# patrickzbhe/ray-tracing-series-rust

Hardware: AMD Instinct MI355X
Metric: Msamples/s (pixels x spp) on Book-1 final scene (higher is better)
Workload: dtype f64

## Files before the change

### ray-tracing-series-rust_amd/csrc/hip/pass_items.inc

```

struct ShardMap {
  int32_t width, block_rows, shard_index, shard_count;
};
struct ActiveMap : ShardMap {
  const uint32_t* active;
};
__device__ __forceinline__ uint32_t map_pixel(const ShardMap&, uint32_t k) { return k; }
__device__ __forceinline__ uint32_t map_pixel(const ActiveMap& m, uint32_t k) { return m.active[k]; }
__device__ __forceinline__ void shard_pixel(const ShardMap& m, uint32_t lp, uint32_t* i, uint32_t* j) {
  uint32_t lr = lp / (uint32_t)m.width;
  *i = lp - lr * (uint32_t)m.width;
  uint32_t k = lr / (uint32_t)m.block_rows;
  uint32_t within = lr - k * (uint32_t)m.block_rows;
  *j = (k * (uint32_t)m.shard_count + (uint32_t)m.shard_index) * (uint32_t)m.block_rows + within;
}

template <class SM>
__device__ __forceinline__ uint32_t item_pixel(const SM& sm, uint32_t npix, uint32_t g, uint32_t* i, uint32_t* j) {
  const uint32_t s_local = g / npix;
  shard_pixel(sm, map_pixel(sm, g - s_local * npix), i, j);
  return s_local;
}

template <class SM>
__device__ __forceinline__ void start_path(const rt::RenderParams& rp, const SM& sm, uint32_t npix, uint32_t s_begin,
                                           uint32_t g, rt::PathState* ps) {
  uint32_t i, j;
  const uint32_t s_local = item_pixel(sm, npix, g, &i, &j);
  rt::path_begin(rp, i, j, s_begin + s_local, ps);
}

__device__ __forceinline__ void store_sample(double* samples, uint32_t g, const rt::Color& c) {
  double* o = samples + 3 * (size_t)g;
  o[0] = c.x; o[1] = c.y; o[2] = c.z;
}

#define TRACE_CHUNK 512u

__device__ __forceinline__ uint32_t lane_rank(unsigned long long mask) {
  return __builtin_amdgcn_mbcnt_hi((uint32_t)(mask >> 32), __builtin_amdgcn_mbcnt_lo((uint32_t)mask, 0u));
}

__device__ __forceinline__ uint32_t queue_claim(unsigned int* work_counter, uint32_t chunk) {
  uint32_t base = 0;
  if ((threadIdx.x & 63u) == 0u) base = atomicAdd(work_counter, chunk);
  return __builtin_amdgcn_readfirstlane(base);
}

#define RING_F64 9u
__host__ __device__ constexpr uint32_t ring_bytes(uint32_t cap) { return cap * (RING_F64 * 8u + 4u); }
```

### ray-tracing-series-rust_amd/csrc/hip/render.hip

```cpp
#include <hip/hip_runtime.h>
#include <cstdio>
#include <cstdlib>
#include <algorithm>
#include <chrono>
#include <cfloat>
#include <cmath>
#include <cstring>
#include <new>
#include <type_traits>
#include <utility>
#include <string>
#include <vector>
#include "../../../include/rtx_abi.h"
#include "../core/cull32.hpp"
#include "../core/integrator.hpp"
#include "../host/flat_scene.hpp"
#include "../host/light_table.hpp"
#include "device_buffer.hpp"
#include "f32_bridge.hpp"
#ifndef RTX_F32_TU
#include "abi_internal.hpp"
#else
namespace rtx { void set_error(const std::string& msg); }
#endif

namespace rtx {

#include "pass_items.inc"

struct FlatNode4;
typedef const FlatNode4 FlatNode4Dev;
struct WorldDesc;

struct LdsSceneDims {
  uint32_t n_nodes, n_refs, n_spheres, n_moving;
  uint32_t node_dwords;
  uint32_t n_uni;
};

struct VoteTop {
  int32_t n;
  int32_t all_rects;
  int32_t k[8];
  uint32_t ref[8];
  rt::FlatRect rect[8];
};

enum class ForcedKernel { none, simple, vote, world, wavefront };

struct TraceSwitches {
  ForcedKernel kernel = ForcedKernel::none;
  bool diag = false;
  int ring = -1, wide = -1, scene_lds = -1;
  bool vote_top = true, tri_direct = true, mat_lds = true, perlin_lds = true;
  bool mv_common = true, motion = true, motion_axis = true;
  bool single_leaf = true, pass_pipeline = true, validate = false;
  uint32_t chunk = TRACE_CHUNK;
  uint32_t world_threshold = 8;
  uint32_t walk_threshold = 0, regen_min = 0, leaf_weight = 0;
  uint32_t wf_paths = 1u << 22, wf_refill = 16, wf_check = 8;
  int wf_occ = 4;
  bool wf_verbose = false;
};

struct Workspace {
  DeviceBuffer<double> samples;
  DeviceBuffer<double> accum;
  DeviceBuffer<rt::TraceCounters> counters;
  DeviceBuffer<unsigned int> work_counter;
  DeviceBuffer<unsigned long long> diag;
  hipEvent_t ev[2] = {nullptr, nullptr};
  hipStream_t aux_stream = nullptr;
  hipEvent_t ev_pass[3] = {nullptr, nullptr, nullptr};
  DeviceBuffer<unsigned char> wave_mem;
  uint32_t* wave_host_ctrl = nullptr;
};

struct VotePlan {
  bool ok = false;
  int32_t bvh_pos = 0;
  int32_t tri_base = -1;
  VoteTop top;
  int blocks_per_cu[2] = {1, 1};
  bool ring[2] = {false, false};
  uint32_t tables = 0;
  size_t tables_bytes = 0;
};

struct WidePlan {
  FlatNode4Dev* nodes4 = nullptr;
  int levels = 0;
  int vote_blocks_per_cu = 1;
};

struct WorldPlan {
  const WorldDesc* desc = nullptr;
  uint32_t mat_lds = 0, tex_lds = 0;
  uint32_t perlin_lds = 0;
  int blocks_per_cu[5][2] = {{1, 1}, {1, 1}, {1, 1}, {1, 1}, {1, 1}};
};

struct LdsFit {
  bool ok = false;
  uint32_t ring_cap = 0;
  uint32_t levels = 0;
  LdsSceneDims dims = {0, 0, 0, 0, 0, 0};
};

struct LdsPlan {
  LdsFit plain;
  LdsFit motion;
  int motion_axis = -1;
  double motion_t0 = 0.0, motion_t1 = 0.0;
  bool mv_common = false;
  double mv_t0 = 0.0, mv_t1 = 1.0;
};

struct WalkTuning {
  uint32_t walk_threshold = 18;
  uint32_t regen_min = 1;
  uint32_t leaf_weight = 3;
  bool single_leaf = false;
};

struct DeviceScene {
  int device = -1;
  std::vector<DeviceBuffer<void>> allocations;
  rt::SceneView view;
  size_t scene_bytes = 0;
  int n_cu = 256;
  double gravity_time_limit = 1e300;
  TraceSwitches sw;
  Workspace ws;
  VotePlan vote;
  WidePlan wide;
  WorldPlan world;
  LdsPlan lds;
  WalkTuning walk;
  rt::LightView lights = {nullptr, nullptr, 0, 0};
};

#define HIP_TRY(expr)                                                                      \
  do {                                                                                     \
    hipError_t _e = (expr);                                                                \
    if (_e != hipSuccess) {                                                                \
      set_error(std::string(#expr) + ": " + hipGetErrorString(_e));                        \
      return RTX_EHIP;                                                                     \
    }                                                                                      \
  } while (0)

template <class T>
static rtx_status upload_array(DeviceScene* ds, const std::vector<T>& v, const T** out) {
  *out = nullptr;
  if (v.empty()) return RTX_OK;
  DeviceBuffer<void> b;
  size_t bytes = v.size() * sizeof(T);
  HIP_TRY(b.alloc(bytes));
  HIP_TRY(hipMemcpy(b, v.data(), bytes, hipMemcpyHostToDevice));
  ds->scene_bytes += bytes;
  *out = (const T*)(void*)b;
  ds->allocations.push_back(std::move(b));
  return RTX_OK;
}

static void free_device_scene(DeviceScene* ds) {
  if (!ds) return;
  Workspace& ws = ds->ws;
  if (ws.wave_host_ctrl) (void)hipHostFree(ws.wave_host_ctrl);
  for (int i = 0; i < 2; ++i)
    if (ws.ev[i]) (void)hipEventDestroy(ws.ev[i]);
  for (int i = 0; i < 3; ++i)
    if (ws.ev_pass[i]) (void)hipEventDestroy(ws.ev_pass[i]);
  if (ws.aux_stream) (void)hipStreamDestroy(ws.aux_stream);
  delete ds;
}

template <class T>
__device__ __forceinline__ T dev_load_uniform(const T* p) { return *(const __attribute__((address_space(4))) T*)(p); }

__device__ __forceinline__ unsigned long long wave_ballot(bool p) { return __builtin_amdgcn_ballot_w64(p); }

#define TRACE_BLOCK 256
struct LdsStack {
  int32_t* base;
  int n;
  static constexpr bool kBottom = false;
  __device__ __forceinline__ void reset() { n = 0; }
  __device__ __forceinline__ void push(int32_t v) { base[n * TRACE_BLOCK] = v; ++n; }
  __device__ __forceinline__ int32_t pop() { --n; return base[n * TRACE_BLOCK]; }
  __device__ __forceinline__ bool empty() const { return n == 0; }
};
// ... 275 lines not shown
  if (a.preset == 0) { LAUNCH_VOTE(P_SPHERES); }
  else { LAUNCH_VOTE(P_MESH); }
#undef LAUNCH_VOTE
#undef LAUNCH_VOTE2
#undef LAUNCH_VOTE3
  return RTX_OK;
}

static void validate_wide_tree(const FlatScene& fs, const std::vector<FlatNode4>& wide, int levels) {
  for (const rt::FlatEntry& e : fs.entries) {
    if (e.kind != rt::ENTRY_BVH) continue;
    std::vector<std::pair<int32_t, int>> todo;
    todo.push_back({e.a, 0});
    size_t visited = 0, bad = 0; int deepest = 0;
    while (!todo.empty()) {
      auto [code, below] = todo.back(); todo.pop_back();
      if (code < 0) { if (rt::leaf_first(code) + rt::leaf_count(code) > (uint32_t)e.c) ++bad; continue; }
      if ((size_t)code >= wide.size()) { ++bad; continue; }
      ++visited;
      int nk = 0;
      for (int k = 0; k < 4; ++k) if (wide[code].child[k] != 0x7fffffff) ++nk;
      deepest = std::max(deepest, below + nk);
      for (int k = 0; k < 4; ++k) if (wide[code].child[k] != 0x7fffffff) todo.push_back({wide[code].child[k], below + nk - 1});
    }
    fprintf(stderr, "[rtx] RTX_VALIDATE: BVH root %d refs %d: %zu wide nodes walked, %zu bad codes, deepest stack %d of %d levels, sizeof(real) %zu\n",
            e.a, e.c, visited, bad, deepest, levels, sizeof(rt::real));
  }
}

static rtx_status plan_wide(DeviceScene* ds, const FlatScene& fs) {
  WidePlan& p = ds->wide;
  const bool spheres_preset = (fs.features & ~P_SPHERES) == 0;
  const bool mesh_preset = !spheres_preset && (fs.features & ~P_MESH) == 0;
  const int preset = spheres_preset ? 0 : (mesh_preset ? 1 : 2);
  const bool for_vote = ds->vote.ok && mesh_preset;
  const bool for_world = !(ds->vote.ok && preset < 2) && preset >= 1;
  bool want_wide = (for_vote && fs.nodes.size() >= 4096) || (for_world && fs.nodes.size() >= 256);
  if (ds->sw.wide >= 0) want_wide = (for_vote || for_world) && ds->sw.wide != 0 && !fs.nodes.empty();
  if (fs.features & rt::F_INSTANCE) want_wide = false;
  if (!want_wide) return RTX_OK;
  std::vector<FlatNode4> wide(fs.nodes.size());
  memset(wide.data(), 0, wide.size() * sizeof(FlatNode4));
  int peak = 0;
  for (const rt::FlatEntry& e : fs.entries)
    if (e.kind == rt::ENTRY_BVH) peak = std::max(peak, build_wide_nodes(fs.nodes, e.a, &wide));
  p.levels = peak + 1;
  const size_t lds = stack_bytes((uint32_t)p.levels);
  bool ok = lds <= 64 * 1024;
  if (ok && for_vote) {
    const int nb = occupancy(k_trace_vote<P_MESH, false, false, true>, lds);
    ok = nb > 0;
    if (ok) p.vote_blocks_per_cu = nb;
  }
  if (ok) {
    rtx_status st = upload_array(ds, wide, &p.nodes4);
    if (st != RTX_OK) return st;
  }
  if (ds->sw.wide >= 0) fprintf(stderr, "[rtx] RTX_WIDE: 4-wide tree %s (%d stack levels)\n", p.nodes4 ? "on" : "off", p.levels);
  if (ds->sw.validate) validate_wide_tree(fs, wide, p.levels);
  return RTX_OK;
}

static rtx_status plan_world(DeviceScene* ds, const FlatScene& fs) {
  WorldPlan& p = ds->world;
  const TraceSwitches& sw = ds->sw;
  rtx_status st = upload_array(ds, build_world_desc(fs), &p.desc);
  if (st != RTX_OK) return st;
  for (int wd = 0; wd < 2; ++wd) {
    const uint32_t levels = (uint32_t)(wd ? ds->wide.levels : fs.max_stack + 1);
    size_t wl = stack_bytes(levels) + (size_t)WORLD_SLOT_F64 * TRACE_BLOCK * sizeof(rt::real);
    if (wl > 64 * 1024) continue;
    if ((wd != 0) == (ds->wide.nodes4 != nullptr)) {
      const size_t n_p = fs.perlins.size();
      if (n_p >= 1 && n_p <= 2 && sw.perlin_lds && wl + n_p * sizeof(rt::FlatPerlin) <= 52 * 1024) {
        p.perlin_lds = (uint32_t)n_p;
        wl += n_p * sizeof(rt::FlatPerlin);
      }
      const size_t mt = fs.materials.size() * sizeof(rt::FlatMaterial) + fs.textures.size() * sizeof(rt::FlatTexture);
      if (!fs.materials.empty() && !fs.textures.empty() && fs.materials.size() <= 64 && fs.textures.size() <= 64 && sw.mat_lds &&
          wl + mt <= 52 * 1024) {
        p.mat_lds = (uint32_t)fs.materials.size();
        p.tex_lds = (uint32_t)fs.textures.size();
        wl += mt;
      }
    }
    int n = 0;
#define WORLD_OCC(I, FEAT) if ((n = occupancy(wd ? k_trace_world<FEAT, true, WORLD_WPS> : k_trace_world<FEAT, false, WORLD_WPS>, wl)) > 0) p.blocks_per_cu[I][wd] = n
    WORLD_OCC(0, P_BOOK2); WORLD_OCC(1, P_ANY); WORLD_OCC(2, P_ALL); WORLD_OCC(3, P_NO_SPHERE_MEDIA);
#undef WORLD_OCC
    if (wd == 0 && (n = occupancy(k_trace_world<P_INST, false, WORLD_WPS>, wl)) > 0) p.blocks_per_cu[4][0] = n;
  }
  return RTX_OK;
}

static rtx_status launch_world(DeviceScene* ds, const PassArgs& a) {
  const WorldPlan& p = ds->world;
  HIP_TRY(hipMemsetAsync(a.work_counter, 0, sizeof(unsigned int), a.stream));
  const bool wide = ds->wide.nodes4 != nullptr;
  const bool book2 = (a.feat & ~P_BOOK2) == 0;
  const bool has_gravity = (a.feat & rt::F_GRAVITY_SPHERE) != 0;
  const bool no_sphere_media = (a.feat & rt::F_MEDIUM_SPHERE) == 0;
  const uint32_t levels = wide ? (uint32_t)ds->wide.levels : a.stack_levels;
  const size_t lds = stack_bytes(levels) + (size_t)WORLD_SLOT_F64 * TRACE_BLOCK * sizeof(rt::real) +
                     (size_t)p.perlin_lds * sizeof(rt::FlatPerlin) + (size_t)p.mat_lds * sizeof(rt::FlatMaterial) +
                     (size_t)p.tex_lds * sizeof(rt::FlatTexture);
  const bool inst = (a.feat & rt::F_INSTANCE) != 0;
  const int family = inst ? 4 : (has_gravity ? 2 : (book2 ? 0 : (no_sphere_media ? 3 : 1)));
  const uint32_t grid = grid_size(a.total, TRACE_BLOCK, (uint64_t)ds->n_cu * (uint64_t)p.blocks_per_cu[family][wide ? 1 : 0]);
  const rt::SceneView& v = ds->view;
#define LAUNCH_WORLD3(FEAT, WIDEF, DIAGF, MAP)                                                                               \
  hipLaunchKernelGGL(HIP_KERNEL_NAME(k_trace_world<FEAT, WIDEF, WORLD_WPS, DIAGF, decltype(MAP)>), dim3(grid), dim3(TRACE_BLOCK), lds, \
                     a.stream, v, a.rp, MAP, a.s_begin, a.total, a.npix, a.samples, a.work_counter, v.entries, v.top_level, v.spheres, \
                     v.moving_spheres, v.rects, v.triangles, v.materials, v.textures, v.refs, ds->wide.nodes4, p.desc,     \
                     ds->walk.leaf_weight, ds->sw.world_threshold, levels, p.perlin_lds, p.mat_lds, p.tex_lds,             \
                     DIAGF ? ds->ws.diag : nullptr)
#define LAUNCH_WORLD2(FEAT, WIDEF) with_map(a, [&](auto map) { LAUNCH_WORLD3(FEAT, WIDEF, false, map); })
#define LAUNCH_WORLD(FEAT) do { if (wide) { LAUNCH_WORLD2(FEAT, true); } else { LAUNCH_WORLD2(FEAT, false); } } while (0)
  if (ds->sw.kernel == ForcedKernel::world && ds->sw.diag && book2 && wide && !a.active) {
    unsigned long long h[24];
    static const char* const names[8] = {"node_step", "leaf_step", "sweep", "shade(lean)", "regen", "direct_entry(all)", "direct_entry(run)", "shade(rare)"};
    return run_diag(ds, a.stream, [&] { LAUNCH_WORLD3(P_BOOK2, true, true, a.sm); }, "world_diag", 18, names, 8, h);
  }
  if (inst) {
    if (wide) { set_error("render: a world with an instance tree has no 4-wide tree"); return RTX_EUNSUPPORTED; }
    LAUNCH_WORLD2(P_INST, false);
  }
  else if (has_gravity) { LAUNCH_WORLD(P_ALL); }
  else if (book2) { LAUNCH_WORLD(P_BOOK2); }
  else if (no_sphere_media) { LAUNCH_WORLD(P_NO_SPHERE_MEDIA); }
  else { LAUNCH_WORLD(P_ANY); }
#undef LAUNCH_WORLD
#undef LAUNCH_WORLD2
#undef LAUNCH_WORLD3
  return RTX_OK;
}

static void fit_lds(LdsFit* f, bool want_ring, uint32_t lds_max) {
  for (uint32_t cap : {64u, 48u, 0u})
    if ((want_ring || cap == 0u) && ldsk_layout(f->levels, cap, f->dims).total <= lds_max) {
      f->ok = true;
      f->ring_cap = cap;
      return;
    }
}

static rtx_status plan_lds(DeviceScene* ds, const FlatScene& fs, const LeafScan& leaves) {
  const bool single_bvh = fs.top_level.size() == 1 && fs.entries[fs.top_level[0]].kind == rt::ENTRY_BVH;
  if (!single_bvh || (fs.features & ~P_SPHERES) != 0 || fs.nodes32.size() > LDSK_MAX_NODES) return RTX_OK;
  LdsPlan& p = ds->lds;
  const TraceSwitches& sw = ds->sw;
  const uint32_t max_end = leaves.max_end, levels = (uint32_t)fs.max_stack + 1u;
  int lds_max = 0;
  (void)hipDeviceGetAttribute(&lds_max, hipDeviceAttributeMaxSharedMemoryPerBlock, ds->device);
  if (lds_max > 160 * 1024) lds_max = 160 * 1024;
  p.plain.levels = levels;
  p.plain.dims = {(uint32_t)fs.nodes32.size(), max_end, max_end, 0u, LDSK_NODE_DWORDS, 0u};
  if (!fs.moving_spheres.empty()) {
    bool same = sw.mv_common;
    for (const rt::FlatMovingSphere& ms : fs.moving_spheres)
      same = same && ms.time0 == fs.moving_spheres[0].time0 && ms.time1 == fs.moving_spheres[0].time1;
    if (same) { p.mv_common = true; p.mv_t0 = (double)fs.moving_spheres[0].time0; p.mv_t1 = (double)fs.moving_spheres[0].time1; }
  }
  if (fs.features & rt::F_MOVING_SPHERE) {
    p.plain.dims.n_uni = (uint32_t)fs.spheres.size();
    p.plain.dims.n_moving = max_end;
    p.plain.dims.n_spheres = 0u;
  }
  p.motion.levels = levels;
  p.motion.dims = p.plain.dims;
  p.motion.dims.node_dwords = LDSK_MOTION_NODE_DWORDS;
  {
    bool moves[3] = {false, false, false};
    for (const rt::FlatMotion32& m : fs.motion32)
      for (int ch = 0; ch < 2; ++ch)
        for (int a = 0; a < 3; ++a) moves[a] = moves[a] || m.dlo[ch][a] != 0.0f || m.dhi[ch][a] != 0.0f;
    if (!fs.motion32.empty() && moves[1] && !moves[0] && !moves[2] && sw.motion_axis) {
      p.motion_axis = 1;
      p.motion.dims.node_dwords = LDSK_MOTION1_NODE_DWORDS;
    }
  }
  if (leaves.max_count <= 4 && max_end <= LDSK_MAX_SLOTS && sw.scene_lds != 0 && lds_max > 0) {
    const bool want_ring = sw.ring != 0;
    fit_lds(&p.plain, want_ring, (uint32_t)lds_max);
    const rt::FlatEntry& be = fs.entries[fs.top_level[0]];
    if (p.plain.ok && !fs.motion32.empty() && (fs.features & rt::F_MOVING_SPHERE) && (double)be.f[0] < (double)be.f[1] && sw.motion) {
      p.motion_t0 = (double)be.f[0]; p.motion_t1 = (double)be.f[1];
      fit_lds(&p.motion, want_ring, (uint32_t)lds_max);
    }
  }
  if (p.plain.ok) {
    hipError_t ae = hipSuccess;
#define LDS_ATTR1(K) if (ae == hipSuccess) ae = hipFuncSetAttribute((const void*)K, hipFuncAttributeMaxDynamicSharedMemorySize, lds_max)
#define LDS_ATTR(FEAT, RINGF, MOTIONF) LDS_ATTR1((k_trace_lds<FEAT, RINGF, MOTIONF>)); LDS_ATTR1((k_trace_lds<FEAT, RINGF, MOTIONF, ActiveMap>))
    LDS_ATTR(P_SPHERES, true, 0u); LDS_ATTR(P_SPHERES, false, 0u); LDS_ATTR(P_STATIC_SPHERES, true, 0u); LDS_ATTR(P_STATIC_SPHERES, false, 0u);
    LDS_ATTR(P_SPHERES, true, 1u); LDS_ATTR(P_SPHERES, false, 1u); LDS_ATTR(P_SPHERES, true, 3u); LDS_ATTR(P_SPHERES, false, 3u);
#undef LDS_ATTR
#undef LDS_ATTR1
    if (ae != hipSuccess) { (void)hipGetLastError(); p.plain.ok = false; }
  }
  if (sw.scene_lds >= 0) {
    auto bytes = [](const LdsFit& f) { return f.ok ? ldsk_layout(f.levels, f.ring_cap, f.dims).total : 0u; };
    fprintf(stderr, "[rtx] RTX_SCENE_LDS: k_trace_lds %s (ring of %u, %u B of LDS); time-aware boxes %s (ring of %u, %u B)\n",
            p.plain.ok ? "on" : "off", p.plain.ring_cap, ldsk_layout(levels, p.plain.ring_cap, p.plain.dims).total,
            p.motion.ok ? "on" : "off", p.motion.ring_cap, bytes(p.motion));
  }
  return RTX_OK;
}

static rtx_status launch_lds(DeviceScene* ds, const PassArgs& a, const RtxCamera* cam) {
  const LdsPlan& p = ds->lds;
  HIP_TRY(hipMemsetAsync(a.work_counter, 0, sizeof(unsigned int), a.stream));
  const bool motion = p.motion.ok && (double)cam->time1 >= p.motion_t0 && (double)cam->time2 <= p.motion_t1;
  const LdsFit& f = motion ? p.motion : p.plain;
  const bool ring = f.ring_cap != 0u;
  const rt::real m_t0 = (rt::real)p.motion_t0, m_inv = (rt::real)(1.0 / (p.motion_t1 - p.motion_t0));
  const LdsKernelLayout L = ldsk_layout(f.levels, f.ring_cap, f.dims);
  const uint32_t grid = grid_size(a.total, LDSK_BLOCK, (uint64_t)ds->n_cu);
  const WalkTuning& wk = ds->walk;
#define LAUNCH_LDS2(FEAT, RINGF, MOTIONF)                                                                               \
  with_map(a, [&](auto map) {                                                                                           \
    hipLaunchKernelGGL(HIP_KERNEL_NAME(k_trace_lds<FEAT, RINGF, MOTIONF, decltype(map)>), dim3(grid), dim3(LDSK_BLOCK), L.total, \
                       a.stream, ds->view, a.rp, map, a.s_begin, a.total, a.npix, a.samples, a.work_counter, wk.leaf_weight, \
                       wk.walk_threshold | (wk.single_leaf ? 0x100u : 0u), ds->sw.chunk, f.ring_cap, f.levels, f.dims,  \
                       m_t0, m_inv, p.mv_common ? 1u : 0u, (rt::real)p.mv_t0, (rt::real)p.mv_t1);                        \
  })
#define LAUNCH_LDS(FEAT, MOTIONF) do { if (ring) { LAUNCH_LDS2(FEAT, true, MOTIONF); } else { LAUNCH_LDS2(FEAT, false, MOTIONF); } } while (0)
  if ((a.feat & ~P_STATIC_SPHERES) == 0) { LAUNCH_LDS(P_STATIC_SPHERES, 0u); }
  else if (motion && p.motion_axis == 1) { LAUNCH_LDS(P_SPHERES, 3u); }
  else if (motion) { LAUNCH_LDS(P_SPHERES, 1u); }
  else { LAUNCH_LDS(P_SPHERES, 0u); }
#undef LAUNCH_LDS
#undef LAUNCH_LDS2
  return RTX_OK;
}

template <bool COUNT>
static void launch_simple(const DeviceScene* ds, const PassArgs& a) {
  const uint32_t grid = grid_size(a.total, TRACE_BLOCK, (uint64_t)ds->n_cu * 8);
#define LAUNCH_SIMPLE2(FEAT, MAP)                                                                                       \
  hipLaunchKernelGGL(HIP_KERNEL_NAME(k_trace_simple<FEAT, COUNT, decltype(MAP)>), dim3(grid), dim3(TRACE_BLOCK), a.stack_lds, \
                     a.stream, ds->view, a.rp, MAP, a.s_begin, a.total, a.npix, a.samples, ds->ws.counters)
#define LAUNCH_SIMPLE(FEAT) with_map(a, [&](auto map) { LAUNCH_SIMPLE2(FEAT, map); })
  const bool inst = (a.feat & rt::F_INSTANCE) != 0;
  if constexpr (COUNT) {
    if (inst) { LAUNCH_SIMPLE2(P_INST, a.sm); } else { LAUNCH_SIMPLE2(P_ALL, a.sm); }
  } else {
    if (a.preset == 0) { LAUNCH_SIMPLE(P_SPHERES); }
    else if (a.preset == 1) { LAUNCH_SIMPLE(P_MESH); }
    else if (inst) { LAUNCH_SIMPLE(P_INST); }
    else { LAUNCH_SIMPLE(P_ALL); }
  }
#undef LAUNCH_SIMPLE
#undef LAUNCH_SIMPLE2
}

#ifndef RTX_F32_TU
static rtx_status launch_nee(const DeviceScene* ds, const PassArgs& a) {
  HIP_TRY(hipMemsetAsync(a.work_counter, 0, sizeof(unsigned int), a.stream));
  const int preset = (a.feat & rt::F_INSTANCE) ? 3 : ((a.feat & ~P_MESH_ROOM) == 0 ? 0 : ((a.feat & rt::F_GRAVITY_SPHERE) ? 2 : 1));
#define LAUNCH_NEE(FEAT, MAP)                                                                                                   \
  do {                                                                                                                          \
    const int nb = occupancy(k_trace_nee<FEAT, decltype(MAP)>, a.stack_lds);                                                    \
    const uint32_t grid = grid_size(a.total, TRACE_CHUNK, (uint64_t)ds->n_cu * (uint64_t)(nb > 0 ? nb : 1) * (TRACE_BLOCK / 64)); \
    hipLaunchKernelGGL(HIP_KERNEL_NAME(k_trace_nee<FEAT, decltype(MAP)>), dim3((grid + TRACE_BLOCK / 64 - 1) / (TRACE_BLOCK / 64)),     \
                       dim3(TRACE_BLOCK), a.stack_lds, a.stream, ds->view, ds->lights, a.rp, MAP, a.s_begin, a.total, a.npix,     \
                       a.samples, a.work_counter);                                                                              \
  } while (0)
  with_map(a, [&](auto map) {
    if (preset == 0) LAUNCH_NEE(P_MESH_ROOM, map);
    else if (preset == 1) LAUNCH_NEE(P_ANY, map);
    else if (preset == 3) LAUNCH_NEE(P_INST, map);
    else LAUNCH_NEE(P_ALL, map);
  });
#undef LAUNCH_NEE
  return RTX_OK;
}
#endif

static rtx_status wave_pass(DeviceScene* ds, const PassArgs& a) {
  Workspace& ws = ds->ws;
  const hipStream_t stream = a.stream;
  uint32_t P = ds->sw.wf_paths;
  if ((uint64_t)P > (uint64_t)a.total) P = a.total;
  P = (P + WF_SEG - 1u) & ~(WF_SEG - 1u);
  const uint32_t n_seg = P / WF_SEG;
  const size_t R = sizeof(rt::real);
  const size_t bytes = 64 + (size_t)P * (16 + 7 * R + 3 * R + 3 * R + R + 4 + 4 + 4 + 4) + (size_t)n_seg * 8;
  HIP_TRY(ws.wave_mem.grow(bytes, stream));
  if (!ws.wave_host_ctrl) HIP_TRY(hipHostMalloc((void**)&ws.wave_host_ctrl, 4 * sizeof(uint32_t), hipHostMallocDefault));
  WavePool pool;
  {
    unsigned char* m = ws.wave_mem;
    pool.ctrl = (uint32_t*)m; m += 64;
    pool.rng = (unsigned long long*)m; m += (size_t)P * 16;
    pool.ray = (rt::real*)m; m += (size_t)P * 7 * R;
    pool.product = (rt::real*)m; m += (size_t)P * 3 * R;
    pool.output = (rt::real*)m; m += (size_t)P * 3 * R;
    pool.hit_t = (rt::real*)m; m += (size_t)P * R;
    pool.depth = (int32_t*)m; m += (size_t)P * 4;
    pool.g = (uint32_t*)m; m += (size_t)P * 4;
    pool.hit_ref = (uint32_t*)m; m += (size_t)P * 4;
    pool.free_list = (uint32_t*)m; m += (size_t)P * 4;
    pool.n_free = (uint32_t*)m; m += (size_t)n_seg * 4;
    pool.cursor = (uint32_t*)m; m += (size_t)n_seg * 4;
    pool.P = P;
  }
  const int preset = a.preset;
  const bool wide = preset == 1 && ds->wide.nodes4 != nullptr;
  const uint32_t levels = wide ? (uint32_t)ds->wide.levels : a.stack_levels;
  const size_t lds = stack_bytes(levels);
  if (lds > 64 * 1024) { set_error("render: BVH too deep for the LDS traversal stack"); return RTX_EUNSUPPORTED; }
  const bool room = (a.feat & ~P_MESH_ROOM) == 0;
  const int occ = ds->sw.wf_occ;
  const uint32_t leaf_weight = ds->walk.leaf_weight, refill = ds->sw.wf_refill, bvh_pos = (uint32_t)ds->vote.bvh_pos;
#define WF_CASES(X)                                                                                                          \
  if (preset == 0) { X(P_SPHERES, false, 4); }                                                                               \
  else if (!wide) { X(P_MESH, false, 4); }                                                                                   \
  else if (room && occ == 5) { X(P_MESH_ROOM, true, 5); }                                                                    \
  else if (room && occ == 6) { X(P_MESH_ROOM, true, 6); }                                                                    \
  else if (room) { X(P_MESH_ROOM, true, 4); }                                                                                \
  else { X(P_MESH, true, 4); }
  int nb = 0;
  hipError_t oe = hipSuccess;
#define WF_OCC(FEAT, WIDEF, MB) oe = hipOccupancyMaxActiveBlocksPerMultiprocessor(&nb, k_wf_trace<FEAT, WIDEF, MB>, TRACE_BLOCK, lds)
  WF_CASES(WF_OCC)
#undef WF_OCC
  if (oe != hipSuccess || nb <= 0) { (void)hipGetLastError(); nb = 1; }
  const uint32_t tgrid = grid_size(P, TRACE_BLOCK, (uint64_t)ds->n_cu * (uint64_t)nb);
  hipLaunchKernelGGL(k_wf_init, dim3((P + 255u) / 256u), dim3(256), 0, stream, pool);
  uint32_t check_every = ds->sw.wf_check;
  int it = 0;
  for (;; ++it) {
    with_map(a, [&](auto map) {
      hipLaunchKernelGGL(HIP_KERNEL_NAME(k_wf_generate<decltype(map)>), dim3(n_seg), dim3(WF_SEG), 0, stream, pool, a.rp, map,
                         a.s_begin, a.total, a.npix);
    });
    if ((uint32_t)(it + 1) % check_every == 0u) {
      HIP_TRY(hipMemsetAsync(pool.ctrl, 0, 16, stream));
      hipLaunchKernelGGL(k_wf_count, dim3(256), dim3(256), 0, stream, pool);
      HIP_TRY(hipGetLastError());
      HIP_TRY(hipMemcpyAsync(ws.wave_host_ctrl, pool.ctrl, 4 * sizeof(uint32_t), hipMemcpyDeviceToHost, stream));
      HIP_TRY(hipStreamSynchronize(stream));
      if (ws.wave_host_ctrl[0] == 0u) break;
      if (ws.wave_host_ctrl[0] < P / 2u) check_every = 2;
      if (it > 100000000) { set_error("render: wavefront integrator did not converge"); return RTX_EHIP; }
    }
#define WF_LAUNCH(FEAT, WIDEF, MB)                                                                                           \
  do {                                                                                                                       \
    hipLaunchKernelGGL(HIP_KERNEL_NAME(k_wf_trace<FEAT, WIDEF, MB>), dim3(tgrid), dim3(TRACE_BLOCK), lds, stream, ds->view, pool, \
                       leaf_weight, refill, bvh_pos, ds->wide.nodes4, ds->vote.tri_base);                                    \
    hipLaunchKernelGGL(HIP_KERNEL_NAME(k_wf_shade<FEAT>), dim3(n_seg), dim3(WF_SEG), 0, stream, ds->view, pool, a.rp, a.samples, bvh_pos); \
// ... 790 lines not shown
```

### ray-tracing-series-rust_amd/csrc/hip/trace_lds.inc

```

#define LDSK_BLOCK 1024
#define LDSK_DONE (-1)
#define LDSK_NO_REF 0xFFFFFFFFu
#define LDSK_MAX_SLOTS 8190u
#define LDSK_MAX_NODES 8191u
#define LDSK_NODE_DWORDS 21u
#ifndef LDSK_NODE_BURST
#define LDSK_NODE_BURST 1
#endif
#define LDSK_MOTION_NODE_DWORDS 39u
#define LDSK_MOTION1_NODE_DWORDS 27u

struct LdsKernelLayout {
  uint32_t off_ring, off_nodes, off_refs, off_spheres, off_moving, total;
};
__host__ __device__ inline LdsKernelLayout ldsk_layout(uint32_t levels, uint32_t ring_cap, const LdsSceneDims& d) {
  LdsKernelLayout L;
  uint32_t o = levels * LDSK_BLOCK * 2u;
  o = (o + 15u) & ~15u;
  L.off_ring = o; o += (LDSK_BLOCK / 64u) * ring_bytes(ring_cap);
  L.off_nodes = o; o += (d.n_nodes * d.node_dwords * 4u + 15u) & ~15u;
  L.off_refs = o;
  L.off_spheres = o; o += (d.n_spheres * (uint32_t)sizeof(rt::FlatSphere) + 15u) & ~15u;
  L.off_moving = o; o += (d.n_moving * (uint32_t)sizeof(rt::FlatMovingSphere) + 15u) & ~15u;
  L.total = o;
  return L;
}

struct LdsStack16 {
  unsigned short* base;
  int n;
  __device__ __forceinline__ void init() { base[0] = 0xFFFFu; n = 1; }
  __device__ __forceinline__ void reset() { n = 1; }
  __device__ __forceinline__ void push(int32_t v) { base[n * LDSK_BLOCK] = (unsigned short)v; ++n; }
  __device__ __forceinline__ int32_t pop() { --n; return (int32_t)(short)base[n * LDSK_BLOCK]; }
  __device__ __forceinline__ int32_t top() const { return (int32_t)(short)base[(n - 1) * LDSK_BLOCK]; }
};
__host__ __device__ __forceinline__ int32_t ldsk_item(int32_t child) {
  if (child >= 0) return child;
  return (int32_t)(short)(unsigned short)(0x8000u | (rt::leaf_first(child) << 2) | (rt::leaf_count(child) - 1u));
}

template <uint32_t F, bool RING, uint32_t MOTION, class SM = ShardMap>
__global__ __launch_bounds__(LDSK_BLOCK) void k_trace_lds(rt::SceneView sv, rt::RenderParams rp, SM sm,
                                                          uint32_t s_begin, uint32_t total, uint32_t npix,
                                                          double* __restrict__ samples, unsigned int* work_counter,
                                                          uint32_t leaf_weight, uint32_t walk_threshold, uint32_t chunk, uint32_t ring_cap,
                                                          uint32_t stack_levels, LdsSceneDims dims, rt::real motion_t0, rt::real motion_inv_dt,
                                                          uint32_t mv_common, rt::real mv_t0, rt::real mv_t1) {
  static_assert(!MOTION || (F & rt::F_MOVING_SPHERE), "time-aware boxes only make sense with moving spheres");
  const bool single_leaf = (walk_threshold & 0x100u) != 0u;
  walk_threshold &= 0xFFu;
  constexpr bool UNI = (F & rt::F_MOVING_SPHERE) != 0;
  constexpr uint32_t FL = UNI ? (F & ~rt::F_SPHERE) : F;
  static_assert(MOTION <= 4u, "0: no slopes, 1: all axes, 2 + a: axis a only");
  constexpr uint32_t ND = MOTION == 1u ? LDSK_MOTION_NODE_DWORDS : (MOTION >= 2u ? LDSK_MOTION1_NODE_DWORDS : LDSK_NODE_DWORDS);
  constexpr uint32_t CBD = MOTION == 1u ? 19u : (MOTION >= 2u ? 13u : 10u);
  constexpr uint32_t MA = MOTION >= 2u ? MOTION - 2u : 0u;
  constexpr uint32_t CB = CBD * 4u;
  constexpr uint32_t ITEM_OFF = CB - 4u;
  static_assert((F & ~(rt::F_SPHERE | rt::F_MOVING_SPHERE | rt::F_BVH | rt::F_LAMBERTIAN | rt::F_METAL |
                       rt::F_DIELECTRIC | rt::F_CHECKER)) == 0, "k_trace_lds caches spheres and moving spheres only");
  extern __shared__ __attribute__((aligned(16))) unsigned char ldsk[];
  const LdsKernelLayout L = ldsk_layout(stack_levels, RING ? ring_cap : 0u, dims);
  const uint32_t lane = threadIdx.x & 63u;
  const rt::FlatEntry& bvh = sv.entries[sv.top_level[0]];
  const int32_t root = bvh.a | (sv.nodes32[bvh.a].axis << 13);
  const uint32_t first_ref = (uint32_t)bvh.b;

  uint32_t* const lds_nodes = (uint32_t*)(ldsk + L.off_nodes);
  rt::FlatSphere* const lds_spheres = (rt::FlatSphere*)(ldsk + L.off_spheres);
  rt::FlatMovingSphere* const lds_moving = (rt::FlatMovingSphere*)(ldsk + L.off_moving);
  {
    static_assert(sizeof(rt::FlatNode32) == 64 && offsetof(rt::FlatNode32, child) == 48 && offsetof(rt::FlatNode32, axis) == 56,
                  "the padded LDS copy assumes FlatNode32's layout");
    const uint32_t* src = (const uint32_t*)sv.nodes32;
    const uint32_t* msrc = (const uint32_t*)sv.motion32;
    for (uint32_t k = threadIdx.x; k < dims.n_nodes * 2u * CBD; k += LDSK_BLOCK) {
      const uint32_t node = k / (2u * CBD), field = k - node * (2u * CBD);
      const uint32_t c = field / CBD, r = field - c * CBD;
      uint32_t v;
      if (r < 9u) {
        const uint32_t a = r / 3u, t = r - a * 3u;
        v = MOTION ? msrc[node * 24u + (t == 1u ? 6u : 0u) + c * 3u + a]
                   : src[node * 16u + (t == 1u ? 6u : 0u) + c * 3u + a];
      } else if (MOTION == 1u && r < 18u) {
        const uint32_t a = (r - 9u) / 3u, t = (r - 9u) - a * 3u;
        v = msrc[node * 24u + (t == 1u ? 18u : 12u) + c * 3u + a];
      } else if (MOTION >= 2u && r < 12u) {
        const uint32_t t = r - 9u;
        v = msrc[node * 24u + (t == 1u ? 18u : 12u) + c * 3u + MA];
      } else {
        const int32_t child = (int32_t)src[node * 16u + 12u + c];
        int32_t item = ldsk_item(child);
        if (child >= 0) item |= sv.nodes32[child].axis << 13;
        v = (uint32_t)item;
      }
      lds_nodes[node * ND + field] = v;
    }
    if (UNI) {
      for (uint32_t k = threadIdx.x; k < dims.n_refs; k += LDSK_BLOCK) {
        const rt::PrimRef ref = sv.refs[first_ref + k];
        rt::FlatMovingSphere m;
        if (rt::primref_type(ref) == rt::PRIM_SPHERE) {
          const rt::FlatSphere sp = sv.spheres[rt::primref_index(ref)];
          m.c0[0] = sp.cx; m.c0[1] = sp.cy; m.c0[2] = sp.cz; m.c1[0] = sp.cx; m.c1[1] = sp.cy; m.c1[2] = sp.cz;
          m.time0 = rt::real(0.0); m.time1 = rt::real(1.0); m.radius = sp.radius; m.mat = sp.mat; m.pad = 0;
        } else {
          m = sv.moving_spheres[rt::primref_index(ref)];
        }
        lds_moving[k] = m;
      }
    } else {
      constexpr uint32_t SD = (uint32_t)(sizeof(rt::FlatSphere) / 4);
      uint32_t* ds = (uint32_t*)lds_spheres;
      const uint32_t* ss = (const uint32_t*)sv.spheres;
      for (uint32_t k = threadIdx.x; k < dims.n_refs * SD; k += LDSK_BLOCK) {
        const uint32_t slot = k / SD, field = k - slot * SD;
        ds[k] = ss[rt::primref_index(sv.refs[first_ref + slot]) * SD + field];
      }
    }
  }
  __syncthreads();
  rt::SceneView lsv = sv;
  lsv.spheres = lds_spheres;
  lsv.moving_spheres = lds_moving;

  LdsStack16 stack;
  stack.base = (unsigned short*)ldsk + threadIdx.x;
  stack.init();
  double* const ring_f = (double*)(ldsk + L.off_ring + (threadIdx.x >> 6) * ring_bytes(ring_cap));
  uint32_t* const ring_g = (uint32_t*)(ring_f + RING_F64 * ring_cap);
  uint32_t ring_n = 0;
  uint32_t chunk_pos = 0, chunk_end = 0;
  bool queue_empty = false;
  bool active = false;
  uint32_t g = 0;
  rt::PathState ps;
  bool midwalk = false;
  rt::Ray32 q = {0.f, 0.f, 0.f, 0.f, 0.f, 0.f, 0.f, 0.f};
  uint32_t dir_neg = 0;
  uint32_t off_x = 0, off_y = 12, off_z = 24;
  uint32_t flip_b = 0;
  float t_max32 = 0.f;
  float s32 = 0.f;
  rt::real mv_ratio = rt::real(0.0);
  int32_t cur = LDSK_DONE;
  rt::Closest best;
  best.t = 0.0; best.ref = LDSK_NO_REF; best.order = 0; best.hit = false;

  for (;;) {
    const unsigned long long need_mask = wave_ballot(!active);
    if (need_mask != 0ull) {
      const uint32_t n_need = (uint32_t)__popcll(need_mask);
      const uint32_t rank = lane_rank(need_mask);
      if (RING) {
#define RING_CAP ring_cap
#define RING_DIAG(mask)
#include "trace_ring.inc"
#undef RING_DIAG
#undef RING_CAP
      } else {
        if (chunk_pos >= chunk_end && !queue_empty) {
          uint32_t base = 0;
          if (lane == 0) base = atomicAdd(work_counter, chunk);
          base = __builtin_amdgcn_readfirstlane(base);
          if (base >= total) {
            queue_empty = true;
          } else {
            chunk_pos = base;
            chunk_end = (total - base < chunk) ? total : base + chunk;
          }
        }
        if (chunk_pos < chunk_end) {
          const uint32_t avail = chunk_end - chunk_pos;
          if (!active && rank < avail) {
            g = chunk_pos + rank;
            start_path(rp, sm, npix, s_begin, g, &ps);
            active = true;
          }
          chunk_pos += (n_need < avail) ? n_need : avail;
        }
      }
    }
    if (wave_ballot(active) == 0ull) break;
    if (active && !midwalk) {
      if (rt::path_bounce_begin(&ps)) {
        store_sample(samples, g, ps.output);
        active = false;
      } else {
        q = rt::make_ray32(ps.ray, rt::ray_t_min(ps.ray));
        dir_neg = rt::ray_dir_neg(ps.ray);
        off_x = (dir_neg & 1u) << 2; off_y = 12u + ((dir_neg & 2u) << 1); off_z = 24u + (dir_neg & 4u);
        flip_b = ((dir_neg & 1u) * CB) | (((dir_neg >> 1) & 1u) * (CB << 8)) | (((dir_neg >> 2) & 1u) * (CB << 16));
        t_max32 = __builtin_huge_valf();
        if (UNI && mv_common != 0u) mv_ratio = (ps.ray.time - mv_t0) / (mv_t1 - mv_t0);
        if (MOTION) s32 = __builtin_fminf(__builtin_fmaxf((float)((ps.ray.time - motion_t0) * motion_inv_dt), 0.f), 1.f);
        best.t = RT_INFINITY; best.ref = LDSK_NO_REF; best.order = 0;
        stack.reset();
        cur = root;
        midwalk = true;
      }
    }
    const uint32_t threshold = (queue_empty && ring_n == 0u) ? 1u : walk_threshold;
    auto node_step = [&]() {
      const unsigned char* nd = (const unsigned char*)(lds_nodes + ((uint32_t)cur & 0x1FFFu) * ND);
      const uint32_t first_b = __builtin_amdgcn_ubfe(flip_b, ((uint32_t)cur >> 10) & 0x18u, 8u);
      const unsigned char* bf = nd + first_b;
      const unsigned char* bs = nd + (CB - first_b);
      const float *fx = (const float*)(bf + off_x), *fy = (const float*)(bf + off_y), *fz = (const float*)(bf + off_z);
      const float *sx = (const float*)(bs + off_x), *sy = (const float*)(bs + off_y), *sz = (const float*)(bs + off_z);
      const int32_t top = stack.top();
      bool hf, hs;
      if (MOTION >= 2u) {
        constexpr uint32_t SO = 9u - 3u * MA;
        const float* fm = MA == 0u ? fx : (MA == 1u ? fy : fz);
        const float* sm = MA == 0u ? sx : (MA == 1u ? sy : sz);
        const float fn = __builtin_fmaf(s32, fm[SO], fm[0]), ff = __builtin_fmaf(s32, fm[SO + 1u], fm[1]);
        const float sn = __builtin_fmaf(s32, sm[SO], sm[0]), sf = __builtin_fmaf(s32, sm[SO + 1u], sm[1]);
        hf = rt::cull32_may_hit_nf_pos(MA == 0u ? fn : fx[0], MA == 0u ? ff : fx[1], MA == 1u ? fn : fy[0], MA == 1u ? ff : fy[1],
                                       MA == 2u ? fn : fz[0], MA == 2u ? ff : fz[1], q, t_max32);
        hs = rt::cull32_may_hit_nf_pos(MA == 0u ? sn : sx[0], MA == 0u ? sf : sx[1], MA == 1u ? sn : sy[0], MA == 1u ? sf : sy[1],
                                       MA == 2u ? sn : sz[0], MA == 2u ? sf : sz[1], q, t_max32);
      } else if (MOTION) {
        hf = rt::cull32_may_hit_nf_pos(__builtin_fmaf(s32, fx[9], fx[0]), __builtin_fmaf(s32, fx[10], fx[1]), __builtin_fmaf(s32, fy[9], fy[0]),
                                   __builtin_fmaf(s32, fy[10], fy[1]), __builtin_fmaf(s32, fz[9], fz[0]), __builtin_fmaf(s32, fz[10], fz[1]), q, t_max32);
        hs = rt::cull32_may_hit_nf_pos(__builtin_fmaf(s32, sx[9], sx[0]), __builtin_fmaf(s32, sx[10], sx[1]), __builtin_fmaf(s32, sy[9], sy[0]),
                                   __builtin_fmaf(s32, sy[10], sy[1]), __builtin_fmaf(s32, sz[9], sz[0]), __builtin_fmaf(s32, sz[10], sz[1]), q, t_max32);
      } else {
        hf = rt::cull32_may_hit_nf_pos(fx[0], fx[1], fy[0], fy[1], fz[0], fz[1], q, t_max32);
        hs = rt::cull32_may_hit_nf_pos(sx[0], sx[1], sy[0], sy[1], sz[0], sz[1], q, t_max32);
      }
      const int32_t cf = *(const int32_t*)(bf + ITEM_OFF), cs = *(const int32_t*)(bs + ITEM_OFF);
      const bool both = hf && hs;
      if (both) stack.base[stack.n * LDSK_BLOCK] = (unsigned short)cs;
      cur = hf ? cf : (hs ? cs : top);
      stack.n += (int)both - (int)!(hf || hs);
    };
    auto leaf_test = [&](uint32_t slot) {
      const rt::PrimRef ref = rt::make_primref(UNI ? rt::PRIM_MOVING_SPHERE : rt::PRIM_SPHERE, slot);
      rt::real t;
      bool ok;
      if (UNI && mv_common != 0u) {
        const rt::FlatMovingSphere& sp = lds_moving[slot];
        const rt::Point3 c0 = rt::load_v3(sp.c0), c1 = rt::load_v3(sp.c1);
        ok = rt::sphere_root(c0 + mv_ratio * (c1 - c0), sp.radius, ps.ray, rt::ray_t_min(ps.ray), best.t, &t);
      } else {
        ok = rt::prim_t<FL, false>(lsv, ref, ps.ray, rt::ray_t_min(ps.ray), best.t, &t, nullptr);
      }
      if (ok && !(t == best.t && slot < best.order)) { best.t = t; best.ref = ref; best.order = slot; }
    };
    for (;;) {
      const bool is_node = cur >= 0;
      const bool is_leaf = cur < -1;
      const uint32_t n_node = (uint32_t)__popcll(wave_ballot(is_node)), n_leaf = (uint32_t)__popcll(wave_ballot(is_leaf));
      if (n_node + n_leaf < threshold) break;
      if (n_node * leaf_weight >= n_leaf) {
        if (is_node) node_step();
#if LDSK_NODE_BURST >= 2
        if (cur >= 0) node_step();
#endif
      } else {
        if (is_leaf) {
          const uint32_t f = ((uint32_t)cur & 0x7FFFu) >> 2;
          if (single_leaf) {
            leaf_test(f);
          } else {
            const uint32_t k = ((uint32_t)cur & 3u) + 1u;
            for (uint32_t i = 0; i < k; ++i) leaf_test(f + i);
          }
          t_max32 = rt::cull_round_up(best.t);
          cur = stack.pop();
        }
      }
    }
    if (midwalk && cur == LDSK_DONE) {
      midwalk = false;
      rt::HitRecord rec;
      const bool hit = best.ref != LDSK_NO_REF;
      if (hit) rt::prim_finalize<FL>(lsv, best.ref, ps.ray, best.t, &rec);
      if (rt::path_bounce_end<F, false>(sv, rp, &ps, hit, rec, nullptr)) {
        store_sample(samples, g, ps.output);
        active = false;
      }
    }
  }
}
```

Baseline: 7861.

## Put LDS node array at offset zero and address traversal through raw LDS pointers

Moves the BVH node array to the start of the dynamic LDS block so node addresses are computed from a constant base. The traversal stack and node loads now use explicit address_space(3) pointers with a byte stack pointer instead of an index. The stack update becomes branch-light: the pointer moves first, then the top is stored conditionally. The walk loop is rotated into a do-while with the ballot at the bottom. A host check disables the LDS kernel if the compiler places static LDS ahead of the node array, which would break the offset-zero assumption. The aim is fewer address computations and generic-pointer overhead in the hot node step, at the risk of falling back to a slower path if static LDS appears.

```diff
diff --git a/ray-tracing-series-rust_amd/csrc/hip/lds_layout.inc b/ray-tracing-series-rust_amd/csrc/hip/lds_layout.inc
--- /dev/null
+++ b/ray-tracing-series-rust_amd/csrc/hip/lds_layout.inc
@@ -0,0 +1,35 @@
+
+#define RING_F64 9u
+__host__ __device__ constexpr uint32_t ring_bytes(uint32_t cap) { return cap * (RING_F64 * 8u + 4u); }
+
+struct LdsSceneDims {
+  uint32_t n_nodes, n_refs, n_spheres, n_moving;
+  uint32_t node_dwords;
+  uint32_t n_uni;
+};
+
+#define LDSK_BLOCK 1024
+#define LDSK_MAX_SLOTS 8190u
+#define LDSK_MAX_NODES 8191u
+#define LDSK_NODE_DWORDS 21u
+#define LDSK_MOTION_NODE_DWORDS 39u
+#define LDSK_MOTION1_NODE_DWORDS 27u
+#define LDSK_OFF_NODES 0u
+#define LDSK_LEVEL_BYTES (LDSK_BLOCK * 2u)
+#define LDSK_LDS_MAX (160u * 1024u)
+
+struct LdsKernelLayout {
+  uint32_t off_nodes, off_refs, off_spheres, off_moving, off_stacks, off_ring, total;
+};
+__host__ __device__ inline LdsKernelLayout ldsk_layout(uint32_t levels, uint32_t ring_cap, const LdsSceneDims& d) {
+  LdsKernelLayout L;
+  uint32_t o = LDSK_OFF_NODES;
+  L.off_nodes = o; o += (d.n_nodes * d.node_dwords * 4u + 15u) & ~15u;
+  L.off_refs = o;
+  L.off_spheres = o; o += (d.n_spheres * (uint32_t)sizeof(rt::FlatSphere) + 15u) & ~15u;
+  L.off_moving = o; o += (d.n_moving * (uint32_t)sizeof(rt::FlatMovingSphere) + 15u) & ~15u;
+  L.off_stacks = o; o += levels * LDSK_LEVEL_BYTES;
+  L.off_ring = o; o += (LDSK_BLOCK / 64u) * ring_bytes(ring_cap);
+  L.total = o;
+  return L;
+}
diff --git a/ray-tracing-series-rust_amd/csrc/hip/pass_items.inc b/ray-tracing-series-rust_amd/csrc/hip/pass_items.inc
--- a/ray-tracing-series-rust_amd/csrc/hip/pass_items.inc
+++ b/ray-tracing-series-rust_amd/csrc/hip/pass_items.inc
@@ -46,6 +46,3 @@
   if ((threadIdx.x & 63u) == 0u) base = atomicAdd(work_counter, chunk);
   return __builtin_amdgcn_readfirstlane(base);
 }
-
-#define RING_F64 9u
-__host__ __device__ constexpr uint32_t ring_bytes(uint32_t cap) { return cap * (RING_F64 * 8u + 4u); }
diff --git a/ray-tracing-series-rust_amd/csrc/hip/render.hip b/ray-tracing-series-rust_amd/csrc/hip/render.hip
--- a/ray-tracing-series-rust_amd/csrc/hip/render.hip
+++ b/ray-tracing-series-rust_amd/csrc/hip/render.hip
@@ -26,17 +26,12 @@
 
 namespace rtx {
 
+#include "lds_layout.inc"
 #include "pass_items.inc"
 
 struct FlatNode4;
 typedef const FlatNode4 FlatNode4Dev;
 struct WorldDesc;
-
-struct LdsSceneDims {
-  uint32_t n_nodes, n_refs, n_spheres, n_moving;
-  uint32_t node_dwords;
-  uint32_t n_uni;
-};
 
 struct VoteTop {
   int32_t n;
@@ -618,7 +613,7 @@
   const uint32_t max_end = leaves.max_end, levels = (uint32_t)fs.max_stack + 1u;
   int lds_max = 0;
   (void)hipDeviceGetAttribute(&lds_max, hipDeviceAttributeMaxSharedMemoryPerBlock, ds->device);
-  if (lds_max > 160 * 1024) lds_max = 160 * 1024;
+  if (lds_max > (int)LDSK_LDS_MAX) lds_max = (int)LDSK_LDS_MAX;
   p.plain.levels = levels;
   p.plain.dims = {(uint32_t)fs.nodes32.size(), max_end, max_end, 0u, LDSK_NODE_DWORDS, 0u};
   if (!fs.moving_spheres.empty()) {
@@ -656,13 +651,22 @@
   }
   if (p.plain.ok) {
     hipError_t ae = hipSuccess;
-#define LDS_ATTR1(K) if (ae == hipSuccess) ae = hipFuncSetAttribute((const void*)K, hipFuncAttributeMaxDynamicSharedMemorySize, lds_max)
+    bool static_lds = false;
+    hipFuncAttributes fa;
+#define LDS_ATTR1(K)                                                                                                   \
+  if (ae == hipSuccess) ae = hipFuncSetAttribute((const void*)K, hipFuncAttributeMaxDynamicSharedMemorySize, lds_max); \
+  if (ae == hipSuccess) ae = hipFuncGetAttributes(&fa, (const void*)K);                                                \
+  if (ae == hipSuccess && fa.sharedSizeBytes != 0) static_lds = true
 #define LDS_ATTR(FEAT, RINGF, MOTIONF) LDS_ATTR1((k_trace_lds<FEAT, RINGF, MOTIONF>)); LDS_ATTR1((k_trace_lds<FEAT, RINGF, MOTIONF, ActiveMap>))
     LDS_ATTR(P_SPHERES, true, 0u); LDS_ATTR(P_SPHERES, false, 0u); LDS_ATTR(P_STATIC_SPHERES, true, 0u); LDS_ATTR(P_STATIC_SPHERES, false, 0u);
     LDS_ATTR(P_SPHERES, true, 1u); LDS_ATTR(P_SPHERES, false, 1u); LDS_ATTR(P_SPHERES, true, 3u); LDS_ATTR(P_SPHERES, false, 3u);
 #undef LDS_ATTR
 #undef LDS_ATTR1
-    if (ae != hipSuccess) { (void)hipGetLastError(); p.plain.ok = false; }
+    if (ae != hipSuccess) { (void)hipGetLastError(); p.plain.ok = false; p.motion.ok = false; }
+    if (static_lds) {
+      fprintf(stderr, "[rtx] k_trace_lds has static LDS in front of its node array: not used\n");
+      p.plain.ok = false; p.motion.ok = false;
+    }
   }
   if (sw.scene_lds >= 0) {
     auto bytes = [](const LdsFit& f) { return f.ok ? ldsk_layout(f.levels, f.ring_cap, f.dims).total : 0u; };
diff --git a/ray-tracing-series-rust_amd/csrc/hip/trace_lds.inc b/ray-tracing-series-rust_amd/csrc/hip/trace_lds.inc
--- a/ray-tracing-series-rust_amd/csrc/hip/trace_lds.inc
+++ b/ray-tracing-series-rust_amd/csrc/hip/trace_lds.inc
@@ -1,40 +1,30 @@
 
-#define LDSK_BLOCK 1024
 #define LDSK_DONE (-1)
 #define LDSK_NO_REF 0xFFFFFFFFu
-#define LDSK_MAX_SLOTS 8190u
-#define LDSK_MAX_NODES 8191u
-#define LDSK_NODE_DWORDS 21u
 #ifndef LDSK_NODE_BURST
 #define LDSK_NODE_BURST 1
 #endif
-#define LDSK_MOTION_NODE_DWORDS 39u
-#define LDSK_MOTION1_NODE_DWORDS 27u
-
-struct LdsKernelLayout {
-  uint32_t off_ring, off_nodes, off_refs, off_spheres, off_moving, total;
-};
-__host__ __device__ inline LdsKernelLayout ldsk_layout(uint32_t levels, uint32_t ring_cap, const LdsSceneDims& d) {
-  LdsKernelLayout L;
-  uint32_t o = levels * LDSK_BLOCK * 2u;
-  o = (o + 15u) & ~15u;
-  L.off_ring = o; o += (LDSK_BLOCK / 64u) * ring_bytes(ring_cap);
-  L.off_nodes = o; o += (d.n_nodes * d.node_dwords * 4u + 15u) & ~15u;
-  L.off_refs = o;
-  L.off_spheres = o; o += (d.n_spheres * (uint32_t)sizeof(rt::FlatSphere) + 15u) & ~15u;
-  L.off_moving = o; o += (d.n_moving * (uint32_t)sizeof(rt::FlatMovingSphere) + 15u) & ~15u;
-  L.total = o;
-  return L;
-}
-
+
+typedef __attribute__((address_space(3))) unsigned char LdsByte;
+typedef __attribute__((address_space(3))) float LdsF32;
+typedef __attribute__((address_space(3))) int32_t LdsI32;
+typedef __attribute__((address_space(3))) short LdsI16;
+typedef __attribute__((address_space(3))) unsigned short LdsU16;
+__device__ __forceinline__ const LdsByte* lds_at(uint32_t addr) { return (const LdsByte*)(uintptr_t)addr; }
 struct LdsStack16 {
-  unsigned short* base;
-  int n;
-  __device__ __forceinline__ void init() { base[0] = 0xFFFFu; n = 1; }
-  __device__ __forceinline__ void reset() { n = 1; }
-  __device__ __forceinline__ void push(int32_t v) { base[n * LDSK_BLOCK] = (unsigned short)v; ++n; }
-  __device__ __forceinline__ int32_t pop() { --n; return (int32_t)(short)base[n * LDSK_BLOCK]; }
-  __device__ __forceinline__ int32_t top() const { return (int32_t)(short)base[(n - 1) * LDSK_BLOCK]; }
+  uint32_t bottom, sp;
+  __device__ __forceinline__ void init() { *(LdsU16*)lds_at(bottom) = 0xFFFFu; sp = bottom; }
+  __device__ __forceinline__ void reset() { sp = bottom; }
+  __device__ __forceinline__ void set_top(int32_t v) { *(LdsU16*)lds_at(sp) = (unsigned short)v; }
+  __device__ __forceinline__ void push(int32_t v) { sp += LDSK_LEVEL_BYTES; set_top(v); }
+  __device__ __forceinline__ int32_t top() const { return (int32_t)*(const LdsI16*)lds_at(sp); }
+  __device__ __forceinline__ int32_t pop() { const int32_t v = top(); sp -= LDSK_LEVEL_BYTES; return v; }
+  __device__ __forceinline__ void move(bool hf, bool hs) {
+    int32_t d = -1;
+    d += (int32_t)hf;
+    d += (int32_t)hs;
+    sp += (uint32_t)d * LDSK_LEVEL_BYTES;
+  }
 };
 __host__ __device__ __forceinline__ int32_t ldsk_item(int32_t child) {
   if (child >= 0) return child;
@@ -68,7 +58,7 @@
   const int32_t root = bvh.a | (sv.nodes32[bvh.a].axis << 13);
   const uint32_t first_ref = (uint32_t)bvh.b;
 
-  uint32_t* const lds_nodes = (uint32_t*)(ldsk + L.off_nodes);
+  uint32_t* const lds_nodes = (uint32_t*)(ldsk + LDSK_OFF_NODES);
   rt::FlatSphere* const lds_spheres = (rt::FlatSphere*)(ldsk + L.off_spheres);
   rt::FlatMovingSphere* const lds_moving = (rt::FlatMovingSphere*)(ldsk + L.off_moving);
   {
@@ -127,7 +117,7 @@
   lsv.moving_spheres = lds_moving;
 
   LdsStack16 stack;
-  stack.base = (unsigned short*)ldsk + threadIdx.x;
+  stack.bottom = (uint32_t)(uintptr_t)(LdsByte*)ldsk + L.off_stacks + threadIdx.x * 2u;
   stack.init();
   double* const ring_f = (double*)(ldsk + L.off_ring + (threadIdx.x >> 6) * ring_bytes(ring_cap));
   uint32_t* const ring_g = (uint32_t*)(ring_f + RING_F64 * ring_cap);
@@ -204,18 +194,18 @@
     }
     const uint32_t threshold = (queue_empty && ring_n == 0u) ? 1u : walk_threshold;
     auto node_step = [&]() {
-      const unsigned char* nd = (const unsigned char*)(lds_nodes + ((uint32_t)cur & 0x1FFFu) * ND);
+      const LdsByte* nd = lds_at(LDSK_OFF_NODES + ((uint32_t)cur & 0x1FFFu) * (ND * 4u));
       const uint32_t first_b = __builtin_amdgcn_ubfe(flip_b, ((uint32_t)cur >> 10) & 0x18u, 8u);
-      const unsigned char* bf = nd + first_b;
-      const unsigned char* bs = nd + (CB - first_b);
-      const float *fx = (const float*)(bf + off_x), *fy = (const float*)(bf + off_y), *fz = (const float*)(bf + off_z);
-      const float *sx = (const float*)(bs + off_x), *sy = (const float*)(bs + off_y), *sz = (const float*)(bs + off_z);
-      const int32_t top = stack.top();
+      const LdsByte* bf = nd + first_b;
+      const LdsByte* bs = nd + (CB - first_b);
+      const LdsF32 *fx = (const LdsF32*)(bf + off_x), *fy = (const LdsF32*)(bf + off_y), *fz = (const LdsF32*)(bf + off_z);
+      const LdsF32 *sx = (const LdsF32*)(bs + off_x), *sy = (const LdsF32*)(bs + off_y), *sz = (const LdsF32*)(bs + off_z);
+      int32_t top = stack.top();
       bool hf, hs;
       if (MOTION >= 2u) {
         constexpr uint32_t SO = 9u - 3u * MA;
-        const float* fm = MA == 0u ? fx : (MA == 1u ? fy : fz);
-        const float* sm = MA == 0u ? sx : (MA == 1u ? sy : sz);
+        const auto* fm = MA == 0u ? fx : (MA == 1u ? fy : fz);
+        const auto* sm = MA == 0u ? sx : (MA == 1u ? sy : sz);
         const float fn = __builtin_fmaf(s32, fm[SO], fm[0]), ff = __builtin_fmaf(s32, fm[SO + 1u], fm[1]);
         const float sn = __builtin_fmaf(s32, sm[SO], sm[0]), sf = __builtin_fmaf(s32, sm[SO + 1u], sm[1]);
         hf = rt::cull32_may_hit_nf_pos(MA == 0u ? fn : fx[0], MA == 0u ? ff : fx[1], MA == 1u ? fn : fy[0], MA == 1u ? ff : fy[1],
@@ -231,11 +221,12 @@
         hf = rt::cull32_may_hit_nf_pos(fx[0], fx[1], fy[0], fy[1], fz[0], fz[1], q, t_max32);
         hs = rt::cull32_may_hit_nf_pos(sx[0], sx[1], sy[0], sy[1], sz[0], sz[1], q, t_max32);
       }
-      const int32_t cf = *(const int32_t*)(bf + ITEM_OFF), cs = *(const int32_t*)(bs + ITEM_OFF);
+      int32_t cf = *(const LdsI32*)(bf + ITEM_OFF), cs = *(const LdsI32*)(bs + ITEM_OFF);
+      asm volatile("" : "+v"(top), "+v"(cf), "+v"(cs));
       const bool both = hf && hs;
-      if (both) stack.base[stack.n * LDSK_BLOCK] = (unsigned short)cs;
       cur = hf ? cf : (hs ? cs : top);
-      stack.n += (int)both - (int)!(hf || hs);
+      stack.move(hf, hs);
+      if (both) stack.set_top(cs);
     };
     auto leaf_test = [&](uint32_t slot) {
       const rt::PrimRef ref = rt::make_primref(UNI ? rt::PRIM_MOVING_SPHERE : rt::PRIM_SPHERE, slot);
@@ -250,28 +241,35 @@
       }
       if (ok && !(t == best.t && slot < best.order)) { best.t = t; best.ref = ref; best.order = slot; }
     };
-    for (;;) {
-      const bool is_node = cur >= 0;
-      const bool is_leaf = cur < -1;
-      const uint32_t n_node = (uint32_t)__popcll(wave_ballot(is_node)), n_leaf = (uint32_t)__popcll(wave_ballot(is_leaf));
-      if (n_node + n_leaf < threshold) break;
-      if (n_node * leaf_weight >= n_leaf) {
-        if (is_node) node_step();
+    {
+      bool is_node = cur >= 0;
+      bool is_leaf = cur < -1;
+      uint32_t n_node = (uint32_t)__popcll(wave_ballot(is_node)), n_leaf = (uint32_t)__popcll(wave_ballot(is_leaf));
+      if (n_node + n_leaf >= threshold) {
+        do {
+          if (n_node * leaf_weight >= n_leaf) {
+            if (is_node) node_step();
 #if LDSK_NODE_BURST >= 2
-        if (cur >= 0) node_step();
+            if (cur >= 0) node_step();
 #endif
-      } else {
-        if (is_leaf) {
-          const uint32_t f = ((uint32_t)cur & 0x7FFFu) >> 2;
-          if (single_leaf) {
-            leaf_test(f);
           } else {
-            const uint32_t k = ((uint32_t)cur & 3u) + 1u;
-            for (uint32_t i = 0; i < k; ++i) leaf_test(f + i);
+            if (is_leaf) {
+              const uint32_t f = ((uint32_t)cur & 0x7FFFu) >> 2;
+              if (single_leaf) {
+                leaf_test(f);
+              } else {
+                const uint32_t k = ((uint32_t)cur & 3u) + 1u;
+                for (uint32_t i = 0; i < k; ++i) leaf_test(f + i);
+              }
+              t_max32 = rt::cull_round_up(best.t);
+              cur = stack.pop();
+            }
           }
-          t_max32 = rt::cull_round_up(best.t);
-          cur = stack.pop();
-        }
+          is_node = cur >= 0;
+          is_leaf = cur < -1;
+          n_node = (uint32_t)__popcll(wave_ballot(is_node));
+          n_leaf = (uint32_t)__popcll(wave_ballot(is_leaf));
+        } while (n_node + n_leaf >= threshold);
       }
     }
     if (midwalk && cur == LDSK_DONE) {
```

New measurement: 8128, median of 6. 1.03x the previous value.
